# yondonfu/ai-rtc-agent

Hardware: NVIDIA H100
Metric: frames/sec at 512x512 SD-Turbo img2img (1-step, stream-batch 1) (higher is better)
Workload: dtype f16

## Files before the change

### ai-rtc-agent_b200/csrc/capi.cu

```cuda
#include "../../include/b200sd.h"

#include "attention.cuh"
#include "codec.cuh"
#include "elementwise.cuh"
#include "igemm.cuh"
#include "tconv.cuh"

using namespace b2;

extern "C" {

const char* b2sd_last_error(void) { return b2_last_error(); }
int b2sd_version(void) { return 1; }

static ActView to_view(const b2sd_act_view& v) {
    ActView a;
    a.ptr = reinterpret_cast<const __half*>(v.ptr);
    a.N = v.n; a.H = v.h; a.W = v.w; a.C = v.c; a.ld = v.ld;
    return a;
}

static void to_igemm_desc(const b2sd_igemm_desc* d, IgemmDesc& g) {
    g.nseg = d->nseg;
    for (int s = 0; s < d->nseg && s < IG_MAX_SRC; ++s) {
// ... 47 lines not shown
    if (igemm_plan(g, &plan)) return -1;
    return igemm_launch(plan, reinterpret_cast<cudaStream_t>(stream));
}

int b2sd_igemm_plan_dry(const b2sd_igemm_desc* d, int autotile, int allow_swap, b2sd_igemm_plan_info* out) {
    if (!d || !out) {
        b2_set_error("b2sd_igemm_plan_dry: null argument");
        return -1;
    }
    IgemmDesc g{};
    to_igemm_desc(d, g);
    g.dbg_ts = nullptr;
    IgemmPlan plan;
    if (autotile == 2) {
        g.max_splits = 4; g.pair_auto = 1; g.pair_splits = 1;
    }
    igemm_set_dry_run(true);
    const int rc = autotile ? igemm_autotile(g, allow_swap != 0, &plan) : igemm_plan(g, &plan);
    igemm_set_dry_run(false);
    if (rc) return -1;
    out->mode = plan.mode;
    out->swap = plan.p.swap;
    out->bn = plan.p.BN;
    out->splits = plan.splits;
    out->grid_x = (int)plan.grid.x; out->grid_y = (int)plan.grid.y; out->grid_z = (int)plan.grid.z;
    out->num_stages = plan.p.num_stages;
    out->acc_bufs = plan.p.acc_bufs;
    out->total_kb = plan.p.total_kb;
    out->kb_per_split = plan.p.kb_per_split;
    out->tmem_cols = (int)plan.p.tmem_cols;
    out->m_tiles = plan.p.tiles_w * plan.p.tiles_h * plan.p.tiles_n;
    out->smem_bytes = (int64_t)plan.smem;
    out->rows_total = plan.rows_total;
    return 0;
}

int b2sd_groupnorm_plan_dry(int ca, int cb, int groups, int hw, int* cluster, int* threads, int* pixels_per_cta) {
    GroupNormArgs a{};
    a.ca = ca; a.cb = cb; a.lda = ca; a.ldb = cb; a.ldy = ca + cb; a.groups = groups; a.hw = hw; a.nb = 1;
    if (groups <= 0 || hw <= 0 || ca <= 0 || !cluster) {
        b2_set_error("b2sd_groupnorm_plan_dry: bad arguments");
        return -1;
    }
    *cluster = groupnorm_plan(a, threads, pixels_per_cta);
    return 0;
}

uint64_t b2sd_igemm_partial_floats(int splits, int64_t rows_total, int n_valid) {
    return igemm_partial_floats(splits, rows_total, n_valid);
}

int b2sd_op_nv12_to_rgb(const void* y, int y_pitch, const void* uv, int uv_pitch, void* rgb_nhwc, int h, int w, int flags, void* stream) {
    return nv12_to_rgb_u8_launch(static_cast<const uint8_t*>(y), y_pitch, static_cast<const uint8_t*>(uv), uv_pitch,
                                 static_cast<uint8_t*>(rgb_nhwc), h, w, flags, reinterpret_cast<cudaStream_t>(stream));
}
int b2sd_op_rgb_to_nv12(const void* rgb_nchw, void* y, int y_pitch, void* uv, int uv_pitch, int h, int w, int flags, void* stream) {
    return rgb_u8_to_nv12_launch(static_cast<const uint8_t*>(rgb_nchw), static_cast<uint8_t*>(y), y_pitch, static_cast<uint8_t*>(uv),
                                 uv_pitch, h, w, flags, reinterpret_cast<cudaStream_t>(stream));
}
int b2sd_codec_probe(void) { return codec_probe(); }

int b2sd_op_attention(const b2sd_attn_desc* d, void* stream) {
    AttnDesc a{};
    a.q = reinterpret_cast<const __half*>(d->q); a.ldq = d->ldq;
    a.k = reinterpret_cast<const __half*>(d->k); a.ldk = d->ldk; a.k_bstride = d->k_bstride; a.k_rows = d->k_rows;
    a.vt = reinterpret_cast<const __half*>(d->vt); a.ldvt = d->ldvt; a.vt_bstride = d->vt_bstride; a.vt_cols = d->vt_cols;
// ... 82 lines not shown
```

### ai-rtc-agent_b200/csrc/igemm.cu

```cuda
#include "igemm.cuh"

#include <cudaTypedefs.h>
#include <stdarg.h>
#include <stdio.h>
#include <stdlib.h>
#include <string.h>

#include "epilogue.cuh"
#include "launch.cuh"
#include "ptx.cuh"

namespace b2 {

#ifdef B2_TIMELINE
#define B2_TS(stmt) stmt
#else
#define B2_TS(stmt)
#endif

static thread_local char g_err[1024] = "";
const char* b2_last_error() { return g_err; }
void b2_set_error(const char* fmt, ...) {
    va_list ap;
    va_start(ap, fmt);
// ... 70 lines not shown
            for (int i = 0; i < 8; ++i) v[i] = fmaxf(v[i], 0.f);
        }
        uint4 o;
        __half2* oh = reinterpret_cast<__half2*>(&o);
#pragma unroll
        for (int i = 0; i < 4; ++i) oh[i] = __floats2half2_rn(v[2 * i], v[2 * i + 1]);
        *reinterpret_cast<uint4*>(e.out + pre.orow[k] * e.ldc + cout0) = o;
    }
}

template <int SPL>
__device__ __forceinline__ void splitk_sum16(uint32_t stg_local, int cc, int row, float (&acc)[16], int rank_mul = 1, int rank_add = 0) {
#pragma unroll
    for (int i = 0; i < 16; ++i) acc[i] = 0.f;
    constexpr int G = SPL < 4 ? SPL : 4;
#pragma unroll
    for (int s0 = 0; s0 < SPL; s0 += G) {
        float4 v[G][4];
#pragma unroll
        for (int s = 0; s < G; ++s) {
            const uint32_t peer = dsmem_map(stg_local, (uint32_t)((s0 + s) * rank_mul + rank_add));
#pragma unroll
            for (int i = 0; i < 4; ++i) v[s][i] = dsmem_ld_f4(peer + (uint32_t)(((cc * 4 + i) * IG_BM + row) * 16));
        }
#pragma unroll
        for (int s = 0; s < G; ++s)
#pragma unroll
            for (int i = 0; i < 4; ++i) {
                acc[4 * i] += v[s][i].x; acc[4 * i + 1] += v[s][i].y; acc[4 * i + 2] += v[s][i].z; acc[4 * i + 3] += v[s][i].w;
            }
    }
}

template <int BN, bool PAIR>
__device__ __forceinline__ void igemm_body(const IgemmParams& p) {
    extern __shared__ uint8_t smem_raw[];
    uint8_t* smem = reinterpret_cast<uint8_t*>((reinterpret_cast<uintptr_t>(smem_raw) + 1023) &
                                               ~static_cast<uintptr_t>(1023));
    const int warp = threadIdx.x >> 5;
    const int lane = threadIdx.x & 31;
    constexpr uint32_t A_BYTES = IG_BM * IG_BK * 2;
    constexpr uint32_t stage_bytes = A_BYTES + (uint32_t)BN * IG_BK * 2;
    uint64_t* full_bar = reinterpret_cast<uint64_t*>(smem + (size_t)p.num_stages * stage_bytes);
    uint64_t* empty_bar = full_bar + IG_MAX_STAGES;
    const int cr = PAIR ? (int)(blockIdx.x & 1) : 0;
    const int mt_first = (int)blockIdx.x;
    const int mt_step = (int)gridDim.x;
    const int mt_guard = PAIR ? cr : 0;

    const int num_mtiles = p.tiles_w * p.tiles_h * p.tiles_n;
    const int ntile = blockIdx.y;
    const int kb_begin = blockIdx.z * p.kb_per_split;
    const int kb_end = min(p.total_kb, kb_begin + p.kb_per_split);
    [[maybe_unused]] unsigned long long* ts = p.dbg_ts ? p.dbg_ts + ((size_t)(blockIdx.z * gridDim.y + blockIdx.y) * gridDim.x + blockIdx.x) * 8 : nullptr;
    B2_TS(if (ts && threadIdx.x == 0) ts[0] = globaltimer_ns();)

    if (threadIdx.x == IG_CONS) {
        for (int s = 0; s < p.nseg; ++s) tma_prefetch_desc(&p.tmA[s]);
        tma_prefetch_desc(&p.tmB);
        for (int s = 0; s < p.num_stages; ++s) {
            mbar_init(&full_bar[s], 1);
            mbar_init(&empty_bar[s], (PAIR ? 2 : 1) * (IG_CONS / 32));
        }
        fence_mbar_init();
    }
    if (PAIR) {
        cluster_arrive_relaxed();
        cluster_wait();
    }
    __syncthreads();

    pdl_launch_dependents();
    pdl_wait();
    B2_TS(if (ts && threadIdx.x == 0) ts[1] = globaltimer_ns();)

    if (warp == IG_CONS / 32) {
        if (lane == 0) {
            [[maybe_unused]] const uint16_t pair_mask = PAIR ? (uint16_t)(3u << (cluster_ctarank() & ~1u)) : (uint16_t)0;
            int stage = 0;
            uint32_t phase = 0;
            for (int mt = mt_first; mt - mt_guard < num_mtiles; mt += mt_step) {
                const int w0 = (mt % p.tiles_w) * p.tw, h0 = ((mt / p.tiles_w) % p.tiles_h) * p.th;
                const int n0 = (mt / (p.tiles_w * p.tiles_h)) * p.tn;
                int seg = 0, base = 0;
                while (seg < p.nseg - 1 && kb_begin >= base + p.seg_ntap[seg] * p.seg_cblocks[seg]) {
                    base += p.seg_ntap[seg] * p.seg_cblocks[seg];
                    ++seg;
                }
                int tap = (kb_begin - base) / p.seg_cblocks[seg];
                int cb = (kb_begin - base) % p.seg_cblocks[seg];
                for (int kb = kb_begin; kb < kb_end; ++kb) {
                    mbar_wait(&empty_bar[stage], phase ^ 1);
#ifdef B2_BOUND_STUDY
                    if (p.dbg_mode == 1 && kb >= kb_begin + p.num_stages) {
                        mbar_arrive(&full_bar[stage]);
                        if (++stage == p.num_stages) { stage = 0; phase ^= 1; }
                        continue;
                    }
#endif
                    mbar_expect_tx(&full_bar[stage], p.a_bytes + p.b_bytes);
                    uint8_t* sa = smem + (size_t)stage * stage_bytes;
                    uint8_t* sb = sa + A_BYTES;
                    int dy = 0, dx = 0;
                    if (p.seg_ntap[seg] == 9) {
                        dy = tap / 3 - 1;
                        dx = tap % 3 - 1;
                    }
                    tma_load_4d(p.swap ? sb : sa, &p.tmA[seg], &full_bar[stage], p.seg_c0[seg] + cb * IG_BK,
                                w0 * p.stride + dx, h0 * p.stride + dy, n0);
                    if (PAIR)
                        tma_load_2d_mc(sb + cr * (BN / 2) * 128, &p.tmB, &full_bar[stage], kb * IG_BK, ntile * BN + cr * (BN / 2), pair_mask);
                    else
                        tma_load_2d(p.swap ? sa : sb, &p.tmB, &full_bar[stage], kb * IG_BK, ntile * (p.swap ? IG_BM : BN));
                    B2_TS(if (ts && mt == (int)blockIdx.x && kb == kb_begin) ts[2] = globaltimer_ns();)
                    if (++cb == p.seg_cblocks[seg]) {
                        cb = 0;
                        if (++tap == p.seg_ntap[seg]) {
                            tap = 0;
                            ++seg;
                        }
                    }
                    if (++stage == p.num_stages) {
                        stage = 0;
                        phase ^= 1;
                    }
                }
            }
        }
    } else {
        const int wg = warp >> 2;
        const int r0 = wg * 64 + (warp & 3) * 16 + (lane >> 2);
        [[maybe_unused]] const uint32_t peer_empty = PAIR ? dsmem_map(smem_u32(empty_bar), cluster_ctarank() ^ 1u) : 0u;
        const IgEpilogue& e = p.epi;
        const bool ln_fma = e.colsum && !p.swap && !(e.flags & IG_SPLITK) && (e.ldc & 7) == 0 && (e.n_valid & 15) == 0;
        const uint32_t smem_base = smem_u32(smem);
        auto release = [&](int s) {
            if (lane == 0) {
                mbar_arrive(&empty_bar[s]);
                if (PAIR) mbar_arrive_remote(peer_empty + (uint32_t)s * 8u);
            }
        };
        int stage = 0;
        uint32_t phase = 0;
        int it = 0;
        for (int mt = mt_first; mt - mt_guard < num_mtiles; mt += mt_step, ++it) {
            float acc[BN / 2];
#pragma unroll
            for (int i = 0; i < BN / 2; ++i) acc[i] = 0.f;
            int prev = -1;
            for (int kb = kb_begin; kb < kb_end; ++kb) {
                mbar_wait(&full_bar[stage], phase);
                B2_TS(if (ts && it == 0 && kb == kb_begin && threadIdx.x == 0) ts[3] = globaltimer_ns();)
                const uint32_t sa = smem_base + (uint32_t)stage * stage_bytes;
                const uint64_t da = make_kmajor_sw128_desc(sa + (uint32_t)wg * (64 * 128));
                const uint64_t db = make_kmajor_sw128_desc(sa + A_BYTES);
#ifdef B2_BOUND_STUDY
                if (p.dbg_mode != 2)
#endif
                {
                    wgmma_fence_regs(acc);
                    wgmma_fence();
#pragma unroll
                    for (int k = 0; k < 4; ++k) Wgmma<BN>::ss(acc, da + 2 * k, db + 2 * k, 1u);
                    wgmma_commit();
                    wgmma_wait<1>();
                    wgmma_fence_regs(acc);
                }
                if (prev >= 0) release(prev);
                prev = stage;
                if (++stage == p.num_stages) {
                    stage = 0;
                    phase ^= 1;
                }
            }
            wgmma_wait<0>();
            wgmma_fence_regs(acc);
            if (prev >= 0) release(prev);
            B2_TS(if (ts && it == 0 && threadIdx.x == 0) ts[4] = globaltimer_ns();)

            const int w0 = (mt % p.tiles_w) * p.tw, h0 = ((mt / p.tiles_w) % p.tiles_h) * p.th;
            const int n0 = (mt / (p.tiles_w * p.tiles_h)) * p.tn;
            if (p.swap || (e.flags & IG_SPLITK)) {
                float* stg = reinterpret_cast<float*>(smem);
// ... 82 lines not shown
            const int t = threadIdx.x;
            const int chunks = BN >> 4;
            const uint32_t stg_local = smem_u32(smem);
            for (int item = t; item < rows_per * chunks; item += IG_CONS) {
                const int rl = item % rows_per;
                const int cc = item / rows_per;
                const int r = rank * rows_per + rl;
                const int wi = r % p.tw, hi = (r / p.tw) % p.th, ni = r / (p.tw * p.th);
                const int n = n0 + ni, h = h0 + hi, w = w0 + wi;
                const bool ok = (ni < p.tn) && (n < p.Nb) && (h < p.Ho) && (w < p.Wo);
                float acc[16];
                switch (splits) {
                    case 2: splitk_sum16<2>(stg_local, cc, r, acc, rk_mul, rk_add); break;
                    case 4: splitk_sum16<4>(stg_local, cc, r, acc, rk_mul, rk_add); break;
                    default: splitk_sum16<8>(stg_local, cc, r, acc, rk_mul, rk_add); break;
                }
                if (ok) {
                    const long orow = ((long)n * p.Ho + h) * p.Wo + w;
                    float mu, rstd;
                    ln_row_stats(p.epi, orow, true, mu, rstd);
                    epi_store16<0>(p.epi, acc, n, orow, ntile * BN + cc * 16, mu, rstd);
                }
            }
        }
        B2_TS(if (ts && threadIdx.x == 0) ts[7] = globaltimer_ns();)
        cluster_sync_all();
    }
    if (PAIR) {
        cluster_arrive_relaxed();
        cluster_wait();
    }
}

template <int BN, bool PAIR>
__global__ void __launch_bounds__(IG_THREADS, 1) igemm_kernel(const __grid_constant__ IgemmParams p) { igemm_body<BN, PAIR>(p); }

using IgemmFn = void (*)(IgemmParams);
template <bool PAIR>
static IgemmFn igemm_fn(int bn) {
    switch (bn) {
#define B2_IG_CASE(N) case N: if constexpr (PAIR && (N % 32)) return nullptr; else return igemm_kernel<N, PAIR>;
        B2_IG_CASE(16) B2_IG_CASE(32) B2_IG_CASE(48) B2_IG_CASE(64) B2_IG_CASE(80) B2_IG_CASE(96) B2_IG_CASE(112) B2_IG_CASE(128)
        B2_IG_CASE(144) B2_IG_CASE(160) B2_IG_CASE(176) B2_IG_CASE(192) B2_IG_CASE(208) B2_IG_CASE(224) B2_IG_CASE(240) B2_IG_CASE(256)
#undef B2_IG_CASE
        default: return nullptr;
    }
}

static PFN_cuTensorMapEncodeTiled_v12000 get_encode() {
    static PFN_cuTensorMapEncodeTiled_v12000 fn = nullptr;
    if (fn) return fn;
    void* p = nullptr;
    cudaDriverEntryPointQueryResult qres;
    cudaError_t err = cudaGetDriverEntryPoint("cuTensorMapEncodeTiled", &p, cudaEnableDefault, &qres);
    if (err != cudaSuccess || qres != cudaDriverEntryPointSuccess || !p) {
        b2_set_error("cudaGetDriverEntryPoint(cuTensorMapEncodeTiled) failed: %s",
                     cudaGetErrorString(err));
        return nullptr;
    }
    fn = reinterpret_cast<PFN_cuTensorMapEncodeTiled_v12000>(p);
    return fn;
}

static thread_local bool g_plan_dry = false;
void igemm_set_dry_run(bool on) { g_plan_dry = on; }

static int encode_act_map(CUtensorMap* m, const ActView& a, int box_c, int box_w, int box_h, int box_n,
                          int estride) {
    if (g_plan_dry) return 0;
    auto enc = get_encode();
    if (!enc) return -1;
    cuuint64_t dims[4] = {(cuuint64_t)a.C, (cuuint64_t)a.W, (cuuint64_t)a.H, (cuuint64_t)a.N};
    cuuint64_t strides[3] = {(cuuint64_t)a.ld * 2, (cuuint64_t)a.W * a.ld * 2,
                             (cuuint64_t)a.H * a.W * a.ld * 2};
    cuuint32_t box[4] = {(cuuint32_t)box_c, (cuuint32_t)box_w, (cuuint32_t)box_h, (cuuint32_t)box_n};
    cuuint32_t es[4] = {1, (cuuint32_t)estride, (cuuint32_t)estride, 1};
    CUresult r = enc(m, CU_TENSOR_MAP_DATA_TYPE_FLOAT16, 4, const_cast<__half*>(a.ptr), dims, strides,
                     box, es, CU_TENSOR_MAP_INTERLEAVE_NONE, CU_TENSOR_MAP_SWIZZLE_128B,
                     CU_TENSOR_MAP_L2_PROMOTION_L2_256B, CU_TENSOR_MAP_FLOAT_OOB_FILL_NONE);
// ... 114 lines not shown
        const size_t need = (splits > 1 ? (size_t)BN * IG_BM * 4 : 0) + (size_t)(cols_per < SWAP_CH ? cols_per : SWAP_CH) * IG_BM * 4;
        if (need > pipe_bytes) {
            stages = (int)((need + stage_bytes - 1) / stage_bytes);
            if (stages > IG_MAX_STAGES) {
                b2_set_error("igemm(swap): split-K staging does not fit (BN %d)", BN);
                return -1;
            }
            pipe_bytes = stages * stage_bytes;
        }
    }
    p.num_stages = stages;
    plan->smem = pipe_bytes + 1024 + 512;
    uint32_t cols = 32;
    while (cols < (uint32_t)BN) cols <<= 1;
    p.tmem_cols = cols;
    plan->grid = dim3(p.tiles_w * p.tiles_h * p.tiles_n, c_tiles, splits);
    plan->mode = 0;
    return 0;
}

int b2_device_sms() {
    static int sms = 0;
    if (sms == 0) {
        int dev = 0, n = 0;
        if (cudaGetDevice(&dev) == cudaSuccess && cudaDeviceGetAttribute(&n, cudaDevAttrMultiProcessorCount, dev) == cudaSuccess && n > 0)
            sms = n;
        else
            sms = IG_SMS;
        cudaGetLastError();
    }
    return sms;
}

static int igemm_ctas_per_sm(int bn, bool pair) {
    if (g_plan_dry) return 1;
    IgemmFn fn = pair ? igemm_fn<true>(bn) : igemm_fn<false>(bn);
    int n = 0;
    if (fn && cudaOccupancyMaxActiveBlocksPerMultiprocessor(&n, fn, IG_THREADS, 0) == cudaSuccess && n > 0) return n;
    cudaGetLastError();
    return 1;
}

int igemm_plan(const IgemmDesc& d, IgemmPlan* plan) {
    *plan = IgemmPlan{};
    if (d.swap) return plan_swap(d, plan);
    IgemmParams& p = plan->p;
    if (d.nseg < 1 || d.nseg > IG_MAX_SRC) {
        b2_set_error("igemm: bad nseg %d", d.nseg);
        return -1;
    }
    const bool geglu = (d.epi.flags & IG_GEGLU) != 0;
    const int n_gemm = geglu ? d.epi.n_valid * 2 : d.epi.n_valid;
    int BN = d.BN;
    if (BN <= 0) {
        if (n_gemm <= 256 && n_gemm % 16 == 0) BN = n_gemm;
        else if (n_gemm < 16) BN = 16;
        else if (n_gemm % 128 == 0) BN = 128;
        else if (n_gemm % 160 == 0) BN = 160;
        else if (n_gemm % 64 == 0) BN = 64;
        else BN = 128;
    }
    if (BN % 16 != 0 || BN < 16 || BN > 256 || (geglu && (BN % 32 != 0 || n_gemm % BN != 0))) {
        b2_set_error("igemm: unsupported BN %d (n %d)", BN, n_gemm);
        return -1;
    }
    const bool pair = d.pair != 0;
    if (pair && BN % 32 != 0) {
        b2_set_error("igemm(pair): BN %d must be a multiple of 32", BN);
        return -1;
    }
    p.BN = BN;
    { static const char* dm = getenv("B2_DBG_MODE"); p.dbg_mode = dm ? atoi(dm) : 0; }
    const int n_tiles = (n_gemm + BN - 1) / BN;
    if (d.w_rows < n_gemm) {
        if (d.w_rows <= 0) {
            b2_set_error("igemm: w_rows %d", d.w_rows);
            return -1;
        }
    }
    int tw, th, tn;
    if (d.Ho == 1 && d.Nb == 1) {
        tw = IG_BM; th = 1; tn = 1;
    } else {
        if (d.Wo <= 16) tw = d.Wo;
        else if (d.Wo % 16 == 0) tw = 16;
        else if (d.Wo % 8 == 0) tw = 8;
        else tw = 16;
        th = IG_BM / tw;
        if (th > d.Ho) th = d.Ho;
        tn = IG_BM / (tw * th);
        if (tn > d.Nb) tn = d.Nb;
        if (tn < 1) tn = 1;
    }
    p.tw = tw; p.th = th; p.tn = tn;
    p.tiles_w = (d.Wo + tw - 1) / tw;
    p.tiles_h = (d.Ho + th - 1) / th;
    p.tiles_n = (d.Nb + tn - 1) / tn;
    p.Wo = d.Wo; p.Ho = d.Ho; p.Nb = d.Nb;
    p.stride = d.stride < 1 ? 1 : d.stride;
    if (p.stride > 2) {
        b2_set_error("igemm: stride %d", p.stride);
        return -1;
    }
    p.nseg = d.nseg;
    int total_kb = 0;
    for (int s = 0; s < d.nseg; ++s) {
        const ActView& a = d.src[s];
        if (a.C % IG_BK != 0 || (a.ld % 8) != 0 || (reinterpret_cast<uintptr_t>(a.ptr) & 15)) {
            b2_set_error("igemm: source %d: C=%d must be a multiple of 64, ld=%d multiple of 8, ptr "
                         "16B aligned",
                         s, a.C, a.ld);
            return -1;
        }
        if (d.ntap[s] != 1 && d.ntap[s] != 9) {
            b2_set_error("igemm: ntap %d", d.ntap[s]);
            return -1;
        }
        p.seg_ntap[s] = d.ntap[s];
        p.seg_cblocks[s] = a.C / IG_BK;
        p.seg_c0[s] = 0;
        total_kb += d.ntap[s] * p.seg_cblocks[s];
        if (encode_act_map(&p.tmA[s], a, IG_BK, tw * p.stride, th * p.stride, tn, p.stride)) return -1;
    }
    p.total_kb = total_kb;
    if (d.w_ld < total_kb * IG_BK || (d.w_ld % 8) != 0 || (reinterpret_cast<uintptr_t>(d.w) & 15)) {
        b2_set_error("igemm: weight ld %d < K %d or misaligned", d.w_ld, total_kb * IG_BK);
        return -1;
    }
    const int b_rows = pair ? BN / 2 : BN;
    if (encode_w_map(&p.tmB, d.w, d.w_rows, d.w_ld, b_rows)) return -1;
    p.a_bytes = (uint32_t)(tw * th * tn) * IG_BK * 2;
    p.b_bytes = (uint32_t)BN * IG_BK * 2;
    int splits = d.splits < 1 ? 1 : d.splits;
    if (splits > total_kb) splits = total_kb;
    if (pair && splits > 4) splits = 4;
    if (splits >= 8) splits = 8;
    else if (splits >= 4) splits = 4;
    else if (splits >= 2) splits = 2;
    p.kb_per_split = (total_kb + splits - 1) / splits;
    while (splits > 1 && (total_kb + p.kb_per_split - 1) / p.kb_per_split != splits) {
        splits >>= 1;
        p.kb_per_split = (total_kb + splits - 1) / splits;
    }
    plan->splits = splits;
    plan->rows_total = (long)d.Nb * d.Ho * d.Wo;
    p.epi = d.epi;
    p.dbg_ts = d.dbg_ts;
    p.n_pad = n_tiles * BN;
    if (splits > 1) {
        if (geglu) {
            b2_set_error("igemm: split-K cannot be combined with GEGLU");
            return -1;
        }
        p.epi.flags |= IG_SPLITK;
    }
    const size_t stage_bytes = (size_t)IG_BM * IG_BK * 2 + (size_t)BN * IG_BK * 2;
    const int per_sm = igemm_ctas_per_sm(BN, pair);
    const long resident = (long)per_sm * b2_device_sms();
    static const char* pc_env = getenv("B2_PERSIST_CTAS");
    const long persist_ctas = pc_env ? atoi(pc_env) : resident;
    const long all_tiles = (long)p.tiles_w * p.tiles_h * p.tiles_n * n_tiles;
    static const bool no_persist_e = getenv("B2_NO_PERSIST") != nullptr;
    const bool will_persist = !no_persist_e && splits == 1 && all_tiles > resident && 2 * BN <= 512;
    const long total_ctas = will_persist ? persist_ctas : all_tiles * splits;
    static const char* stage_env = getenv("B2_STAGE_KB");
    const size_t ring_budget = stage_env ? (size_t)atoi(stage_env) * 1024
                                         : (d.ring_kb > 0 ? (size_t)d.ring_kb * 1024
                                                          : (size_t)((per_sm >= 2 && total_ctas > b2_device_sms() ? 100 : 200) * 1024));
    int stages = (int)(ring_budget / stage_bytes);
    if (stages < 2) stages = 2;
    if (stages > IG_MAX_STAGES) stages = IG_MAX_STAGES;
    if (stages > p.kb_per_split) stages = p.kb_per_split < 2 ? 2 : p.kb_per_split;
    p.num_stages = stages;
    size_t pipe_bytes = stages * stage_bytes;
    if (splits > 1) {
        const size_t stg = (size_t)BN * IG_BM * 4;
        if (stg > pipe_bytes) {
            stages = (int)((stg + stage_bytes - 1) / stage_bytes);
            if (stages > IG_MAX_STAGES) {
                b2_set_error("igemm: split-K staging does not fit (BN %d)", BN);
                return -1;
            }
            p.num_stages = stages;
            pipe_bytes = stages * stage_bytes;
        }
    }
    plan->smem = pipe_bytes + 1024  + 512 ;
    const int m_tiles = p.tiles_w * p.tiles_h * p.tiles_n;
    int grid_x = m_tiles;
    p.acc_bufs = 1;
    if (will_persist) {
        grid_x = (int)(persist_ctas / n_tiles);
        if (grid_x < 1) grid_x = 1;
        if (grid_x > m_tiles) grid_x = m_tiles;
        p.acc_bufs = 2;
    }
    if (pair) {
        grid_x = (p.acc_bufs == 2 && grid_x > 2) ? (grid_x & ~1) : ((grid_x + 1) & ~1);
    }
    uint32_t cols = 32;
    while (cols < (uint32_t)(BN * p.acc_bufs)) cols <<= 1;
    p.tmem_cols = cols;
    plan->grid = dim3(grid_x, n_tiles, splits);
    plan->mode = pair ? 1 : 0;
    plan->pair = pair ? 1 : 0;
    return 0;
}

int igemm_encode_act_map(CUtensorMap* m, const ActView& a, int box_c, int box_w, int box_h, int box_n, int estride) {
    return encode_act_map(m, a, box_c, box_w, box_h, box_n, estride);
}
int igemm_encode_w_map(CUtensorMap* m, const __half* w, int rows, int ld, int box_rows) { return encode_w_map(m, w, rows, ld, box_rows); }

int igemm_init() {
    static bool attr_set = false;
    if (!attr_set) {
        for (int bn = 16; bn <= 256; bn += 16) {
            for (int pair = 0; pair < 2; ++pair) {
                IgemmFn fn = pair ? igemm_fn<true>(bn) : igemm_fn<false>(bn);
                if (!fn) continue;
                cudaError_t e = cudaFuncSetAttribute(fn, cudaFuncAttributeMaxDynamicSharedMemorySize, 227 * 1024);
                if (e != cudaSuccess) {
                    b2_set_error("cudaFuncSetAttribute(igemm BN %d%s): %s", bn, pair ? " pair" : "", cudaGetErrorString(e));
                    return -1;
                }
            }
        }
        if (!get_encode()) return -1;
        attr_set = true;
    }
    return 0;
}

int igemm_launch(const IgemmPlan& plan, cudaStream_t stream) {
    if (igemm_init()) return -1;
    const int cz = plan.splits > 1 ? plan.splits : 1;
    IgemmFn fn = plan.pair ? igemm_fn<true>(plan.p.BN) : igemm_fn<false>(plan.p.BN);
    if (!fn) {
        b2_set_error("igemm launch: no kernel for BN %d%s", plan.p.BN, plan.pair ? " (CTA pair)" : "");
        return -1;
    }
    cudaError_t e = plan.pair ? launch_kc(fn, plan.grid, dim3(IG_THREADS), plan.smem, stream, 2, cz, plan.p)
                              : launch_k(fn, plan.grid, dim3(IG_THREADS), plan.smem, stream, cz, plan.p);
    if (e != cudaSuccess) {
        b2_set_error("igemm launch: %s", cudaGetErrorString(e));
        return -1;
    }
    return 0;
}

}
```

### ai-rtc-agent_b200/csrc/igemm.cuh

```cuda
#pragma once
#include <cuda.h>
#include <cuda_fp16.h>
#include <cuda_runtime.h>
#include <stdint.h>

namespace b2 {

constexpr int IG_BM = 128;
constexpr int IG_BK = 64;
constexpr int IG_MAX_SRC = 3;
constexpr int IG_MAX_STAGES = 8;
constexpr int IG_CONS = 256;
constexpr int IG_THREADS = IG_CONS + 32;
constexpr int IG_SMS = 132;

enum : int {
    IG_RELU = 1,
    IG_GEGLU = 2,
    IG_SPLITK = 4,
};

struct IgEpilogue {
    __half* out;
    int ldc;
    const float* colbias;
    int colbias_bstride;
    const __half* res;
    int ldr;
    float acc_scale;
    float res_scale;
    int flags;
    int n_valid;
    unsigned long long* rowstat_out;
    const unsigned long long* rowstat_in;
    const float* colsum;
    float ln_inv_c, ln_eps;
    __half* out2;
    int ld2, col2;
};

constexpr float IG_STAT_SCALE = 1048576.f;

struct IgemmParams {
    CUtensorMap tmA[IG_MAX_SRC];
    CUtensorMap tmB;
    int seg_ntap[IG_MAX_SRC];
    int seg_cblocks[IG_MAX_SRC];
    int seg_c0[IG_MAX_SRC];
    int nseg;
    int total_kb;
    int kb_per_split;
    int tw, th, tn;
    int tiles_w, tiles_h, tiles_n;
    int Wo, Ho, Nb;
    int stride;
    int BN;
    int num_stages;
    int acc_bufs;
    uint32_t a_bytes;
    uint32_t b_bytes;
    uint32_t tmem_cols;
    unsigned long long* dbg_ts;
    int n_pad;
    int swap;
    int tw_log2, th_log2;
    int dbg_mode;
    IgEpilogue epi;
};

struct ActView {
    const __half* ptr;
    int N, H, W, C;
    int ld;
};

struct IgemmDesc {
    ActView src[IG_MAX_SRC];
    int ntap[IG_MAX_SRC];
    int nseg;
    const __half* w;
    int w_rows;
    int w_ld;
    int stride;
    int Nb, Ho, Wo;
    int BN;
    int swap;
    int splits;
    int ring_kb;
    int max_splits;
    int pair_auto;
    int pair_splits;
    int pair;
    unsigned long long* dbg_ts;
    float* partial;
    int* tile_counters;
    IgEpilogue epi;
};

struct IgemmPlan {
// ... 22 lines not shown
```

### ai-rtc-agent_b200/host/capi.py

```python
from __future__ import annotations

import ctypes as C
import os

_HERE = os.path.dirname(os.path.abspath(__file__))
LIB_PATH = os.environ.get("B200SD_LIB") or os.path.join(os.path.dirname(_HERE), "libb200sd.so")


class B2Error(RuntimeError):
    pass


class ActView(C.Structure):
    _fields_ = [("ptr", C.c_void_p), ("n", C.c_int), ("h", C.c_int), ("w", C.c_int), ("c", C.c_int),
                ("ld", C.c_int)]


class IgemmDesc(C.Structure):
    _fields_ = [
        ("src", ActView * 3), ("ntap", C.c_int * 3), ("nseg", C.c_int),
        ("w", C.c_void_p), ("w_rows", C.c_int), ("w_ld", C.c_int), ("stride", C.c_int),
        ("nb", C.c_int), ("ho", C.c_int), ("wo", C.c_int),
        ("bn", C.c_int), ("splits", C.c_int), ("partial", C.c_void_p),
        ("out", C.c_void_p), ("ldc", C.c_int),
        ("colbias", C.c_void_p), ("colbias_bstride", C.c_int),
        ("res", C.c_void_p), ("ldr", C.c_int),
        ("acc_scale", C.c_float), ("res_scale", C.c_float),
        ("flags", C.c_int), ("n_valid", C.c_int), ("swap", C.c_int),
        ("rowstat_out", C.c_void_p), ("rowstat_in", C.c_void_p), ("colsum", C.c_void_p), ("ln_c", C.c_int), ("ln_eps", C.c_float),
        ("out2", C.c_void_p), ("ld2", C.c_int), ("col2", C.c_int),
    ]


class IgemmPlanInfo(C.Structure):
    _fields_ = [
        ("mode", C.c_int), ("swap", C.c_int), ("bn", C.c_int), ("splits", C.c_int),
        ("grid_x", C.c_int), ("grid_y", C.c_int), ("grid_z", C.c_int),
        ("num_stages", C.c_int), ("acc_bufs", C.c_int), ("total_kb", C.c_int), ("kb_per_split", C.c_int),
        ("tmem_cols", C.c_int), ("m_tiles", C.c_int),
        ("smem_bytes", C.c_int64), ("rows_total", C.c_int64),
    ]


class AttnDesc(C.Structure):
    _fields_ = [
        ("q", C.c_void_p), ("ldq", C.c_int),
        ("k", C.c_void_p), ("ldk", C.c_int), ("k_bstride", C.c_int64), ("k_rows", C.c_int64),
        ("vt", C.c_void_p), ("ldvt", C.c_int), ("vt_bstride", C.c_int64), ("vt_cols", C.c_int64),
        ("out", C.c_void_p), ("ldo", C.c_int),
        ("nb", C.c_int), ("heads", C.c_int), ("sq", C.c_int), ("skv", C.c_int), ("d_real", C.c_int),
        ("dp", C.c_int),
    ]


class EngineConfig(C.Structure):
    _fields_ = [
        ("block_out_channels", C.c_int * 4), ("heads", C.c_int * 4), ("down_attn", C.c_int * 4),
        ("cross_attention_dim", C.c_int), ("layers_per_block", C.c_int), ("norm_groups", C.c_int),
        ("ctx_tokens", C.c_int), ("batch", C.c_int), ("height", C.c_int), ("width", C.c_int),
        ("do_add_noise", C.c_int), ("use_cuda_graph", C.c_int),
    ]


IN_U8_NHWC, IN_F32_NCHW, IN_F16_NCHW = 0, 1, 2
OUT_U8_NCHW, OUT_F16_NCHW = 0, 1
IG_RELU = 1
IG_GEGLU = 2
IG_TCONV = 64
IG_PAIR = 128

_lib = None


# ... 70 lines not shown
```

### include/b200sd.h

```cpp
#ifndef B200SD_H
#define B200SD_H

#include <stdint.h>

#ifdef __cplusplus
extern "C" {
#endif

const char* b2sd_last_error(void);
int b2sd_version(void);


typedef struct {
    const void* ptr;
    int n, h, w, c;
    int ld;
} b2sd_act_view;

enum {
    B2SD_IG_RELU = 1,
    B2SD_IG_GEGLU = 2,
    B2SD_IG_TCONV = 64,
    B2SD_IG_PAIR = 128
};
// ... 10 lines not shown
    int splits;
    void* partial;
    void* out;
    int ldc;
    const float* colbias;
    int colbias_bstride;
    const void* res;
    int ldr;
    float acc_scale, res_scale;
    int flags;
    int n_valid;
    int swap;
    void* rowstat_out;
    const void* rowstat_in;
    const float* colsum;
    int ln_c;
    float ln_eps;
    void* out2;
    int ld2, col2;
} b2sd_igemm_desc;

int b2sd_op_igemm(const b2sd_igemm_desc* d, void* stream);

typedef struct {
    int mode;
    int swap, bn, splits;
    int grid_x, grid_y, grid_z;
    int num_stages;
    int acc_bufs;
    int total_kb, kb_per_split;
    int tmem_cols;
    int m_tiles;
    int64_t smem_bytes, rows_total;
} b2sd_igemm_plan_info;
int b2sd_igemm_plan_dry(const b2sd_igemm_desc* d, int autotile, int allow_swap, b2sd_igemm_plan_info* out);

int b2sd_groupnorm_plan_dry(int ca, int cb, int groups, int hw, int* cluster, int* threads, int* pixels_per_cta);
uint64_t b2sd_igemm_partial_floats(int splits, int64_t rows_total, int n_valid);

typedef struct {
    const void* q; int ldq;
    const void* k; int ldk; int64_t k_bstride; int64_t k_rows;
    const void* vt; int ldvt; int64_t vt_bstride; int64_t vt_cols;
    void* out; int ldo;
    int nb, heads, sq, skv, d_real, dp;
} b2sd_attn_desc;
int b2sd_op_attention(const b2sd_attn_desc* d, void* stream);

int b2sd_op_groupnorm(const void* xa, int ca, int lda, const void* xb, int cb, int ldb, const float* gamma,
                      const float* beta, void* y, int ldy, int nb, int hw, int groups, float eps, int silu,
                      void* stream);
int b2sd_groupnorm_last_path(void);
int b2sd_op_layernorm(const void* x, int ldx, const float* gamma, const float* beta, void* y, int ldy,
                      int64_t rows, int c, float eps, void* stream);
int b2sd_op_upsample2x(const void* x, void* y, int nb, int h, int w, int c, void* stream);
int b2sd_op_smallconv(const void* x, const void* w_oihw, const float* bias, void* y, int ldy, int nb, int h,
                      int w, int cin, int cout, int in_h, int in_w, int flags, void* stream);
int b2sd_op_lcm_step(void* x, const void* eps, const void* noise, const float* coef, void* out_latent, int T,
                     int hw, int do_add_noise, void* stream);
enum { B2SD_CSC_BT601 = 1, B2SD_CSC_FULL_RANGE = 2 };
int b2sd_op_nv12_to_rgb(const void* y, int y_pitch, const void* uv, int uv_pitch, void* rgb_nhwc, int h, int w, int flags, void* stream);
int b2sd_op_rgb_to_nv12(const void* rgb_nchw, void* y, int y_pitch, void* uv, int uv_pitch, int h, int w, int flags, void* stream);
int b2sd_codec_probe(void);
int b2sd_op_post_u8(const void* y_nhwc, int ldy, void* out_nchw_u8, int nb, int h, int w, void* stream);

typedef struct b2sd_engine* b2sd_handle;
// ... 52 lines not shown
```

Baseline: 176.8.

## Load halo activation tile once per channel block and reuse across 3x3 taps

Adds a HALO variant of the implicit-GEMM conv kernel. For stride-1 3x3 convolutions without split-K it loads a (tw+2)x(th+2) activation slab once per channel block into a separate A-slot ring, then runs all nine taps against shifted shared-memory descriptors, so activations are no longer re-fetched by TMA for every tap. Weights stream through their own ring. The cost is a new set of barriers, a fixed 8x8 or 8x16 tile shape, extra smem for the halo slots, and a shared-memory descriptor stride trick that must match the swizzle layout.

New measurement: 178.0 (median of 6 runs). No clear change (+0.7%).

```diff
diff --git a/ai-rtc-agent_b200/csrc/capi.cu b/ai-rtc-agent_b200/csrc/capi.cu
--- a/ai-rtc-agent_b200/csrc/capi.cu
+++ b/ai-rtc-agent_b200/csrc/capi.cu
@@ -103,6 +103,7 @@
     out->m_tiles = plan.p.tiles_w * plan.p.tiles_h * plan.p.tiles_n;
     out->smem_bytes = (int64_t)plan.smem;
     out->rows_total = plan.rows_total;
+    out->halo = plan.p.halo;
     return 0;
 }
 
diff --git a/ai-rtc-agent_b200/csrc/igemm.cu b/ai-rtc-agent_b200/csrc/igemm.cu
--- a/ai-rtc-agent_b200/csrc/igemm.cu
+++ b/ai-rtc-agent_b200/csrc/igemm.cu
@@ -126,7 +126,7 @@
     }
 }
 
-template <int BN, bool PAIR>
+template <int BN, bool PAIR, bool HALO>
 __device__ __forceinline__ void igemm_body(const IgemmParams& p) {
     extern __shared__ uint8_t smem_raw[];
     uint8_t* smem = reinterpret_cast<uint8_t*>((reinterpret_cast<uintptr_t>(smem_raw) + 1023) &
@@ -134,9 +134,14 @@
     const int warp = threadIdx.x >> 5;
     const int lane = threadIdx.x & 31;
     constexpr uint32_t A_BYTES = IG_BM * IG_BK * 2;
-    constexpr uint32_t stage_bytes = A_BYTES + (uint32_t)BN * IG_BK * 2;
-    uint64_t* full_bar = reinterpret_cast<uint64_t*>(smem + (size_t)p.num_stages * stage_bytes);
+    constexpr uint32_t B_BYTES = (uint32_t)BN * IG_BK * 2;
+    constexpr uint32_t stage_bytes = A_BYTES + B_BYTES;
+    const size_t ring_bytes = HALO ? (size_t)p.a_slots * p.a_slot_bytes + (size_t)p.num_stages * B_BYTES
+                                     : (size_t)p.num_stages * stage_bytes;
+    uint64_t* full_bar = reinterpret_cast<uint64_t*>(smem + ring_bytes);
     uint64_t* empty_bar = full_bar + IG_MAX_STAGES;
+    uint64_t* afull_bar = empty_bar + IG_MAX_STAGES;
+    uint64_t* aempty_bar = afull_bar + IG_MAX_ASLOTS;
     const int cr = PAIR ? (int)(blockIdx.x & 1) : 0;
     const int mt_first = (int)blockIdx.x;
     const int mt_step = (int)gridDim.x;
@@ -156,6 +161,12 @@
             mbar_init(&full_bar[s], 1);
             mbar_init(&empty_bar[s], (PAIR ? 2 : 1) * (IG_CONS / 32));
         }
+        if (HALO) {
+            for (int s = 0; s < p.a_slots; ++s) {
+                mbar_init(&afull_bar[s], 1);
+                mbar_init(&aempty_bar[s], IG_CONS / 32);
+            }
+        }
         fence_mbar_init();
     }
     if (PAIR) {
@@ -173,7 +184,67 @@
             [[maybe_unused]] const uint16_t pair_mask = PAIR ? (uint16_t)(3u << (cluster_ctarank() & ~1u)) : (uint16_t)0;
             int stage = 0;
             uint32_t phase = 0;
-            for (int mt = mt_first; mt - mt_guard < num_mtiles; mt += mt_step) {
+            auto load_b = [&](uint8_t* sb, int kb) {
+                if (PAIR)
+                    tma_load_2d_mc(sb + cr * (BN / 2) * 128, &p.tmB, &full_bar[stage], kb * IG_BK, ntile * BN + cr * (BN / 2), pair_mask);
+                else
+                    tma_load_2d(sb, &p.tmB, &full_bar[stage], kb * IG_BK, ntile * BN);
+            };
+            if constexpr (HALO) {
+                uint8_t* const bring = smem + (size_t)p.a_slots * p.a_slot_bytes;
+                int aslot = 0;
+                uint32_t aphase = 0;
+                for (int mt = mt_first; mt - mt_guard < num_mtiles; mt += mt_step) {
+                    const int w0 = (mt % p.tiles_w) * p.tw, h0 = ((mt / p.tiles_w) % p.tiles_h) * p.th;
+                    const int n0 = (mt / (p.tiles_w * p.tiles_h)) * p.tn;
+                    [[maybe_unused]] int nb_loaded = 0, na_loaded = 0;
+                    int base = 0;
+                    for (int seg = 0; seg < p.nseg; ++seg) {
+                        const int ntap = p.seg_ntap[seg], ncb = p.seg_cblocks[seg];
+                        for (int cb = 0; cb < ncb; ++cb) {
+                            mbar_wait(&aempty_bar[aslot], aphase ^ 1);
+                            bool skip_a = false;
+#ifdef B2_BOUND_STUDY
+                            skip_a = p.dbg_mode == 1 && na_loaded++ >= p.a_slots;
+#endif
+                            if (skip_a) {
+                                mbar_arrive(&afull_bar[aslot]);
+                            } else {
+                                uint8_t* sa = smem + (size_t)aslot * p.a_slot_bytes;
+                                const int c = p.seg_c0[seg] + cb * IG_BK;
+                                mbar_expect_tx(&afull_bar[aslot], ntap == 9 ? p.halo_bytes : p.a_bytes);
+                                if (ntap == 9)
+                                    tma_load_4d(sa, &p.tmA[seg], &afull_bar[aslot], c, w0 - 1, h0 - 1, n0);
+                                else
+                                    tma_load_4d(sa, &p.tmA[seg], &afull_bar[aslot], c, w0, h0, n0);
+                            }
+                            if (++aslot == p.a_slots) {
+                                aslot = 0;
+                                aphase ^= 1;
+                            }
+                            for (int t = 0; t < ntap; ++t) {
+                                mbar_wait(&empty_bar[stage], phase ^ 1);
+                                bool skip_b = false;
+#ifdef B2_BOUND_STUDY
+                                skip_b = p.dbg_mode == 1 && nb_loaded++ >= p.num_stages;
+#endif
+                                if (skip_b) {
+                                    mbar_arrive(&full_bar[stage]);
+                                } else {
+                                    mbar_expect_tx(&full_bar[stage], p.b_bytes);
+                                    load_b(bring + (size_t)stage * B_BYTES, base + t * ncb + cb);
+                                }
+                                if (++stage == p.num_stages) {
+                                    stage = 0;
+                                    phase ^= 1;
+                                }
+                            }
+                        }
+                        base += ntap * ncb;
+                    }
+                }
+            }
+            for (int mt = mt_first; !HALO && mt - mt_guard < num_mtiles; mt += mt_step) {
                 const int w0 = (mt % p.tiles_w) * p.tw, h0 = ((mt / p.tiles_w) % p.tiles_h) * p.th;
                 const int n0 = (mt / (p.tiles_w * p.tiles_h)) * p.tn;
                 int seg = 0, base = 0;
@@ -202,10 +273,10 @@
                     }
                     tma_load_4d(p.swap ? sb : sa, &p.tmA[seg], &full_bar[stage], p.seg_c0[seg] + cb * IG_BK,
                                 w0 * p.stride + dx, h0 * p.stride + dy, n0);
-                    if (PAIR)
-                        tma_load_2d_mc(sb + cr * (BN / 2) * 128, &p.tmB, &full_bar[stage], kb * IG_BK, ntile * BN + cr * (BN / 2), pair_mask);
+                    if (PAIR || !p.swap)
+                        load_b(sb, kb);
                     else
-                        tma_load_2d(p.swap ? sa : sb, &p.tmB, &full_bar[stage], kb * IG_BK, ntile * (p.swap ? IG_BM : BN));
+                        tma_load_2d(sa, &p.tmB, &full_bar[stage], kb * IG_BK, ntile * IG_BM);
                     B2_TS(if (ts && mt == (int)blockIdx.x && kb == kb_begin) ts[2] = globaltimer_ns();)
                     if (++cb == p.seg_cblocks[seg]) {
                         cb = 0;
@@ -236,13 +307,65 @@
         };
         int stage = 0;
         uint32_t phase = 0;
+        int aslot = 0;
+        uint32_t aphase = 0;
+        const int pitch = p.tw + 2;
+        const int hi0 = 8 * wg;
+        const int slab_row0 = (hi0 / p.th) * (p.th + 2) + hi0 % p.th;
+        const uint32_t bring = smem_base + (uint32_t)p.a_slots * p.a_slot_bytes;
         int it = 0;
         for (int mt = mt_first; mt - mt_guard < num_mtiles; mt += mt_step, ++it) {
             float acc[BN / 2];
 #pragma unroll
             for (int i = 0; i < BN / 2; ++i) acc[i] = 0.f;
             int prev = -1;
-            for (int kb = kb_begin; kb < kb_end; ++kb) {
+            if constexpr (HALO) {
+                int prev_a = -1;
+                for (int seg = 0; seg < p.nseg; ++seg) {
+                    const int ntap = p.seg_ntap[seg], ncb = p.seg_cblocks[seg];
+                    for (int cb = 0; cb < ncb; ++cb) {
+                        mbar_wait(&afull_bar[aslot], aphase);
+                        const uint32_t sa = smem_base + (uint32_t)aslot * p.a_slot_bytes;
+                        for (int t = 0; t < ntap; ++t) {
+                            mbar_wait(&full_bar[stage], phase);
+                            const uint64_t da = ntap == 9 ? make_kmajor_sw128_desc(sa + (uint32_t)((slab_row0 + t / 3) * pitch + t % 3) * 128u,
+                                                                                  (uint32_t)pitch * 128u)
+                                                          : make_kmajor_sw128_desc(sa + (uint32_t)wg * (64 * 128));
+                            const uint64_t db = make_kmajor_sw128_desc(bring + (uint32_t)stage * B_BYTES);
+#ifdef B2_BOUND_STUDY
+                            if (p.dbg_mode != 2)
+#endif
+                            {
+                                wgmma_fence_regs(acc);
+                                wgmma_fence();
+#pragma unroll
+                                for (int k = 0; k < 4; ++k) Wgmma<BN>::ss(acc, da + 2 * k, db + 2 * k, 1u);
+                                wgmma_commit();
+                                wgmma_wait<1>();
+                                wgmma_fence_regs(acc);
+                            }
+                            if (prev >= 0) release(prev);
+                            if (prev_a >= 0 && lane == 0) mbar_arrive(&aempty_bar[prev_a]);
+                            prev = stage;
+                            prev_a = t == ntap - 1 ? aslot : -1;
+                            if (++stage == p.num_stages) {
+                                stage = 0;
+                                phase ^= 1;
+                            }
+                        }
+                        if (++aslot == p.a_slots) {
+                            aslot = 0;
+                            aphase ^= 1;
+                        }
+                    }
+                }
+                wgmma_wait<0>();
+                wgmma_fence_regs(acc);
+                if (prev >= 0) release(prev);
+                if (prev_a >= 0 && lane == 0) mbar_arrive(&aempty_bar[prev_a]);
+                prev = -1;
+            }
+            for (int kb = kb_begin; !HALO && kb < kb_end; ++kb) {
                 mbar_wait(&full_bar[stage], phase);
                 B2_TS(if (ts && it == 0 && kb == kb_begin && threadIdx.x == 0) ts[3] = globaltimer_ns();)
                 const uint32_t sa = smem_base + (uint32_t)stage * stage_bytes;
@@ -391,19 +514,23 @@
     }
 }
 
-template <int BN, bool PAIR>
-__global__ void __launch_bounds__(IG_THREADS, 1) igemm_kernel(const __grid_constant__ IgemmParams p) { igemm_body<BN, PAIR>(p); }
+template <int BN, bool PAIR, bool HALO>
+__global__ void __launch_bounds__(IG_THREADS, 1) igemm_kernel(const __grid_constant__ IgemmParams p) { igemm_body<BN, PAIR, HALO>(p); }
 
 using IgemmFn = void (*)(IgemmParams);
-template <bool PAIR>
+template <bool PAIR, bool HALO>
 static IgemmFn igemm_fn(int bn) {
     switch (bn) {
-#define B2_IG_CASE(N) case N: if constexpr (PAIR && (N % 32)) return nullptr; else return igemm_kernel<N, PAIR>;
+#define B2_IG_CASE(N) case N: if constexpr ((PAIR && (N % 32)) || (HALO && N > IG_HALO_MAX_BN)) return nullptr; else return igemm_kernel<N, PAIR, HALO>;
         B2_IG_CASE(16) B2_IG_CASE(32) B2_IG_CASE(48) B2_IG_CASE(64) B2_IG_CASE(80) B2_IG_CASE(96) B2_IG_CASE(112) B2_IG_CASE(128)
         B2_IG_CASE(144) B2_IG_CASE(160) B2_IG_CASE(176) B2_IG_CASE(192) B2_IG_CASE(208) B2_IG_CASE(224) B2_IG_CASE(240) B2_IG_CASE(256)
 #undef B2_IG_CASE
         default: return nullptr;
     }
+}
+static IgemmFn igemm_kernel_for(int bn, bool pair, bool halo) {
+    return pair ? (halo ? igemm_fn<true, true>(bn) : igemm_fn<true, false>(bn))
+                : (halo ? igemm_fn<false, true>(bn) : igemm_fn<false, false>(bn));
 }
 
 static PFN_cuTensorMapEncodeTiled_v12000 get_encode() {
@@ -584,9 +711,9 @@
     return sms;
 }
 
-static int igemm_ctas_per_sm(int bn, bool pair) {
+static int igemm_ctas_per_sm(int bn, bool pair, bool halo) {
     if (g_plan_dry) return 1;
-    IgemmFn fn = pair ? igemm_fn<true>(bn) : igemm_fn<false>(bn);
+    IgemmFn fn = igemm_kernel_for(bn, pair, halo);
     int n = 0;
     if (fn && cudaOccupancyMaxActiveBlocksPerMultiprocessor(&n, fn, IG_THREADS, 0) == cudaSuccess && n > 0) return n;
     cudaGetLastError();
@@ -630,8 +757,56 @@
             return -1;
         }
     }
+    p.stride = d.stride < 1 ? 1 : d.stride;
+    if (p.stride > 2) {
+        b2_set_error("igemm: stride %d", p.stride);
+        return -1;
+    }
+    p.nseg = d.nseg;
+    int total_kb = 0;
+    bool has9 = false;
+    for (int s = 0; s < d.nseg; ++s) {
+        const ActView& a = d.src[s];
+        if (a.C % IG_BK != 0 || (a.ld % 8) != 0 || (reinterpret_cast<uintptr_t>(a.ptr) & 15)) {
+            b2_set_error("igemm: source %d: C=%d must be a multiple of 64, ld=%d multiple of 8, ptr "
+                         "16B aligned",
+                         s, a.C, a.ld);
+            return -1;
+        }
+        if (d.ntap[s] != 1 && d.ntap[s] != 9) {
+            b2_set_error("igemm: ntap %d", d.ntap[s]);
+            return -1;
+        }
+        p.seg_ntap[s] = d.ntap[s];
+        p.seg_cblocks[s] = a.C / IG_BK;
+        p.seg_c0[s] = 0;
+        total_kb += d.ntap[s] * p.seg_cblocks[s];
+        has9 = has9 || d.ntap[s] == 9;
+    }
+    p.total_kb = total_kb;
+    if (d.w_ld < total_kb * IG_BK || (d.w_ld % 8) != 0 || (reinterpret_cast<uintptr_t>(d.w) & 15)) {
+        b2_set_error("igemm: weight ld %d < K %d or misaligned", d.w_ld, total_kb * IG_BK);
+        return -1;
+    }
+    int splits = d.splits < 1 ? 1 : d.splits;
+    if (splits > total_kb) splits = total_kb;
+    if (pair && splits > 4) splits = 4;
+    if (splits >= 8) splits = 8;
+    else if (splits >= 4) splits = 4;
+    else if (splits >= 2) splits = 2;
+    p.kb_per_split = (total_kb + splits - 1) / splits;
+    while (splits > 1 && (total_kb + p.kb_per_split - 1) / p.kb_per_split != splits) {
+        splits >>= 1;
+        p.kb_per_split = (total_kb + splits - 1) / splits;
+    }
+    p.halo = has9 && p.stride == 1 && splits == 1 && BN <= IG_HALO_MAX_BN && d.Wo >= 8 && d.Ho >= 8;
     int tw, th, tn;
-    if (d.Ho == 1 && d.Nb == 1) {
+    if (p.halo) {
+        tw = 8;
+        th = d.Ho <= 8 ? 8 : 16;
+        tn = IG_BM / (tw * th);
+        if (tn > d.Nb) tn = d.Nb;
+    } else if (d.Ho == 1 && d.Nb == 1) {
         tw = IG_BM; th = 1; tn = 1;
     } else {
         if (d.Wo <= 16) tw = d.Wo;
@@ -649,51 +824,16 @@
     p.tiles_h = (d.Ho + th - 1) / th;
     p.tiles_n = (d.Nb + tn - 1) / tn;
     p.Wo = d.Wo; p.Ho = d.Ho; p.Nb = d.Nb;
-    p.stride = d.stride < 1 ? 1 : d.stride;
-    if (p.stride > 2) {
-        b2_set_error("igemm: stride %d", p.stride);
-        return -1;
-    }
-    p.nseg = d.nseg;
-    int total_kb = 0;
     for (int s = 0; s < d.nseg; ++s) {
-        const ActView& a = d.src[s];
-        if (a.C % IG_BK != 0 || (a.ld % 8) != 0 || (reinterpret_cast<uintptr_t>(a.ptr) & 15)) {
-            b2_set_error("igemm: source %d: C=%d must be a multiple of 64, ld=%d multiple of 8, ptr "
-                         "16B aligned",
-                         s, a.C, a.ld);
+        const bool halo_seg = p.halo && d.ntap[s] == 9;
+        if (encode_act_map(&p.tmA[s], d.src[s], IG_BK, halo_seg ? tw + 2 : tw * p.stride, halo_seg ? th + 2 : th * p.stride, tn,
+                           p.stride))
             return -1;
-        }
-        if (d.ntap[s] != 1 && d.ntap[s] != 9) {
-            b2_set_error("igemm: ntap %d", d.ntap[s]);
-            return -1;
-        }
-        p.seg_ntap[s] = d.ntap[s];
-        p.seg_cblocks[s] = a.C / IG_BK;
-        p.seg_c0[s] = 0;
-        total_kb += d.ntap[s] * p.seg_cblocks[s];
-        if (encode_act_map(&p.tmA[s], a, IG_BK, tw * p.stride, th * p.stride, tn, p.stride)) return -1;
-    }
-    p.total_kb = total_kb;
-    if (d.w_ld < total_kb * IG_BK || (d.w_ld % 8) != 0 || (reinterpret_cast<uintptr_t>(d.w) & 15)) {
-        b2_set_error("igemm: weight ld %d < K %d or misaligned", d.w_ld, total_kb * IG_BK);
-        return -1;
     }
     const int b_rows = pair ? BN / 2 : BN;
     if (encode_w_map(&p.tmB, d.w, d.w_rows, d.w_ld, b_rows)) return -1;
     p.a_bytes = (uint32_t)(tw * th * tn) * IG_BK * 2;
     p.b_bytes = (uint32_t)BN * IG_BK * 2;
-    int splits = d.splits < 1 ? 1 : d.splits;
-    if (splits > total_kb) splits = total_kb;
-    if (pair && splits > 4) splits = 4;
-    if (splits >= 8) splits = 8;
-    else if (splits >= 4) splits = 4;
-    else if (splits >= 2) splits = 2;
-    p.kb_per_split = (total_kb + splits - 1) / splits;
-    while (splits > 1 && (total_kb + p.kb_per_split - 1) / p.kb_per_split != splits) {
-        splits >>= 1;
-        p.kb_per_split = (total_kb + splits - 1) / splits;
-    }
     plan->splits = splits;
     plan->rows_total = (long)d.Nb * d.Ho * d.Wo;
     p.epi = d.epi;
@@ -707,7 +847,7 @@
         p.epi.flags |= IG_SPLITK;
     }
     const size_t stage_bytes = (size_t)IG_BM * IG_BK * 2 + (size_t)BN * IG_BK * 2;
-    const int per_sm = igemm_ctas_per_sm(BN, pair);
+    const int per_sm = igemm_ctas_per_sm(BN, pair, p.halo != 0);
     const long resident = (long)per_sm * b2_device_sms();
     static const char* pc_env = getenv("B2_PERSIST_CTAS");
     const long persist_ctas = pc_env ? atoi(pc_env) : resident;
@@ -737,7 +877,21 @@
             pipe_bytes = stages * stage_bytes;
         }
     }
+    if (p.halo) {
+        p.halo_bytes = (uint32_t)((tw + 2) * (th + 2) * tn) * IG_BK * 2;
+        p.a_slot_bytes = ((p.halo_bytes > p.a_bytes ? p.halo_bytes : p.a_bytes) + 1023u) & ~1023u;
+        const size_t b_ring = (size_t)stages * p.b_bytes;
+        int slots = ring_budget > b_ring ? (int)((ring_budget - b_ring) / p.a_slot_bytes) : 0;
+        if (slots < 2) slots = 2;
+        if (slots > IG_MAX_ASLOTS) slots = IG_MAX_ASLOTS;
+        p.a_slots = slots;
+        pipe_bytes = b_ring + (size_t)slots * p.a_slot_bytes;
+    }
     plan->smem = pipe_bytes + 1024  + 512 ;
+    if (plan->smem > 227 * 1024) {
+        b2_set_error("igemm: operand rings of %zu bytes do not fit shared memory (BN %d, %d stages)", pipe_bytes, BN, stages);
+        return -1;
+    }
     const int m_tiles = p.tiles_w * p.tiles_h * p.tiles_n;
     int grid_x = m_tiles;
     p.acc_bufs = 1;
@@ -768,12 +922,13 @@
     static bool attr_set = false;
     if (!attr_set) {
         for (int bn = 16; bn <= 256; bn += 16) {
-            for (int pair = 0; pair < 2; ++pair) {
-                IgemmFn fn = pair ? igemm_fn<true>(bn) : igemm_fn<false>(bn);
+            for (int v = 0; v < 4; ++v) {
+                const int pair = v & 1, halo = v >> 1;
+                IgemmFn fn = igemm_kernel_for(bn, pair, halo);
                 if (!fn) continue;
                 cudaError_t e = cudaFuncSetAttribute(fn, cudaFuncAttributeMaxDynamicSharedMemorySize, 227 * 1024);
                 if (e != cudaSuccess) {
-                    b2_set_error("cudaFuncSetAttribute(igemm BN %d%s): %s", bn, pair ? " pair" : "", cudaGetErrorString(e));
+                    b2_set_error("cudaFuncSetAttribute(igemm BN %d%s%s): %s", bn, pair ? " pair" : "", halo ? " halo" : "", cudaGetErrorString(e));
                     return -1;
                 }
             }
@@ -787,9 +942,9 @@
 int igemm_launch(const IgemmPlan& plan, cudaStream_t stream) {
     if (igemm_init()) return -1;
     const int cz = plan.splits > 1 ? plan.splits : 1;
-    IgemmFn fn = plan.pair ? igemm_fn<true>(plan.p.BN) : igemm_fn<false>(plan.p.BN);
+    IgemmFn fn = igemm_kernel_for(plan.p.BN, plan.pair, plan.p.halo);
     if (!fn) {
-        b2_set_error("igemm launch: no kernel for BN %d%s", plan.p.BN, plan.pair ? " (CTA pair)" : "");
+        b2_set_error("igemm launch: no kernel for BN %d%s%s", plan.p.BN, plan.pair ? " (CTA pair)" : "", plan.p.halo ? " (halo)" : "");
         return -1;
     }
     cudaError_t e = plan.pair ? launch_kc(fn, plan.grid, dim3(IG_THREADS), plan.smem, stream, 2, cz, plan.p)
diff --git a/ai-rtc-agent_b200/csrc/igemm.cuh b/ai-rtc-agent_b200/csrc/igemm.cuh
--- a/ai-rtc-agent_b200/csrc/igemm.cuh
+++ b/ai-rtc-agent_b200/csrc/igemm.cuh
@@ -10,6 +10,8 @@
 constexpr int IG_BK = 64;
 constexpr int IG_MAX_SRC = 3;
 constexpr int IG_MAX_STAGES = 8;
+constexpr int IG_MAX_ASLOTS = 4;
+constexpr int IG_HALO_MAX_BN = 128;
 constexpr int IG_CONS = 256;
 constexpr int IG_THREADS = IG_CONS + 32;
 constexpr int IG_SMS = 132;
@@ -65,6 +67,10 @@
     int swap;
     int tw_log2, th_log2;
     int dbg_mode;
+    int halo;
+    int a_slots;
+    uint32_t a_slot_bytes;
+    uint32_t halo_bytes;
     IgEpilogue epi;
 };
 
diff --git a/ai-rtc-agent_b200/host/capi.py b/ai-rtc-agent_b200/host/capi.py
--- a/ai-rtc-agent_b200/host/capi.py
+++ b/ai-rtc-agent_b200/host/capi.py
@@ -38,7 +38,7 @@
         ("grid_x", C.c_int), ("grid_y", C.c_int), ("grid_z", C.c_int),
         ("num_stages", C.c_int), ("acc_bufs", C.c_int), ("total_kb", C.c_int), ("kb_per_split", C.c_int),
         ("tmem_cols", C.c_int), ("m_tiles", C.c_int),
-        ("smem_bytes", C.c_int64), ("rows_total", C.c_int64),
+        ("smem_bytes", C.c_int64), ("rows_total", C.c_int64), ("halo", C.c_int),
     ]
 
 
diff --git a/include/b200sd.h b/include/b200sd.h
--- a/include/b200sd.h
+++ b/include/b200sd.h
@@ -66,6 +66,7 @@
     int tmem_cols;
     int m_tiles;
     int64_t smem_bytes, rows_total;
+    int halo;
 } b2sd_igemm_plan_info;
 int b2sd_igemm_plan_dry(const b2sd_igemm_desc* d, int autotile, int allow_swap, b2sd_igemm_plan_info* out);
 
```
